# Wu-sm/Adversarial-Attacks-on-GAN-based-Image-Fusion

Measured on AMD Instinct MI355X. Metric: attacked images/sec, PGD-20 L∞ ε=8/255 at 256², 1/2/4/8 MI355X, higher is better.
Workload: dtype f32; 1 GPU; PGD-20 L∞ eps=8/255 alpha=2/255 at 256², 128 images/GPU (BASELINE config #4 per-GPU share), RCCL all-gather of outputs when N>1; encoder=e4e, norm=linf, images_per_gpu=128, global_batch=128, size=256, pgd_steps=20, parallelism=dp1, dist_world_size=1, output_in_eps_ball_and_finite=True, fp32_arithmetic=fp32

## Files before the change

### adversarial-attacks-on-gan-based-image-fusion_amd/csrc/conv_halo_x6.hip

```cpp
#include <type_traits>

#include "conv_common.h"
#include "halo_epilogue.h"

namespace mia {

#ifdef MIA_STAMPS
__device__ unsigned long long g_x6_stamps[4][24];
#endif

template <int BN_, int TPS_ = 1>
struct HaloX6 {
  static constexpr int PH = 16, PW = 16, NW = 8, NT = 64 * NW;
  static constexpr int WN = BN_ == 128 ? 2 : 1, WM = NW / WN, FM = 16 / WM, FN = 4;
  static constexpr int BM = PH * PW, BN = BN_, BK = 32;
  static constexpr int HSIDE = PW + 2, HROWS = (PH + 2) * HSIDE;
  static constexpr int HPIECES = (HROWS + 7) / 8;
  static constexpr int HBUF = HPIECES * 1024;
  static constexpr int LROWB = 64, LBUF = HROWS * LROWB;
  static constexpr int TPS = TPS_, NG = (9 + TPS - 1) / TPS;
  static constexpr int BHM = BN * ROWB, BL = BN * LROWB, BSTAGE1 = BHM + BL;
  static constexpr int BSTAGE = TPS * BSTAGE1;
  static constexpr int BWAVES = 4, HWAVES = 4;
  static constexpr int B_HM_INS = BN / 8 / BWAVES;
// ... 2 lines not shown
  static constexpr int HSTEPS = (4 + TPS - 1) / TPS;
  static constexpr int H_PER_STEP = (H_INS + HSTEPS - 1) / HSTEPS;
  static constexpr int EROWS = 128, ES = BN + 4;
  static constexpr int LDS = 2 * HBUF + LBUF + 2 * BSTAGE;
  static_assert(WM * FM * 16 == BM && WN * FN * 16 == BN, "");
  static_assert(B_HM_INS * 8 * BWAVES == BN && B_L_INS * 16 * BWAVES == BN, "");
  static_assert(LDS <= 160 * 1024, "");
};

template <int BN_, bool PRO, int EPI, bool EARLY, bool PRIO, bool UNR, int TPS = 1, int STG = 0>
__global__ __launch_bounds__(HaloX6<BN_>::NT, 2) void conv_halo_x6_kernel(const ConvK k) {
  static_assert(!UNR || (EARLY && PRIO && EPI != -2), "UNR: the EARLY + PRIO schedule, D[ch][px]");
  static_assert(UNR || TPS == 1, "several taps per K-step: the unrolled loop only");
  static_assert(STG == 0 || (UNR && TPS == 1 && BN_ == 128), "staggered loop: the 128-column tile");
  typedef HaloX6<BN_, TPS> TL;
  constexpr int NG = TL::NG;
  constexpr int FM = TL::FM, FN = TL::FN, WN = TL::WN, NT = TL::NT, BN = TL::BN, BK = TL::BK;
  constexpr int HSIDE = TL::HSIDE, HROWS = TL::HROWS, HPIECES = TL::HPIECES, HBUF = TL::HBUF;
  constexpr int H_INS = TL::H_INS, HPS = TL::H_PER_STEP, HWAVES = TL::HWAVES;
  constexpr int B_HM_INS = TL::B_HM_INS, B_L_INS = TL::B_L_INS, BSTAGE = TL::BSTAGE;

  extern __shared__ __attribute__((aligned(16))) char smem[];
  char* const hbuf = smem;
  char* const lbuf = smem + 2 * HBUF;
  char* const bring = lbuf + TL::LBUF;

  const mia_conv_args& p = k.a;
  const int tid = threadIdx.x, lane = tid & 63;
  const int wid = __builtin_amdgcn_readfirstlane(tid >> 6);
  const int wm = wid / WN, wn = wid % WN;
  const ConvGroup G = k.g[0];
  const int H = p.H, W = p.W, Cin = p.Cin, Cout = p.Cout, Kpad = G.kpad;
  const int bl = xcd_remap(blockIdx.x, k.nblk);
  const int mt = bl / k.nbn, n0 = (bl % k.nbn) * BN;
  const int ptx = W / TL::PW, pty = H / TL::PH;
  const int x0 = (mt % ptx) * TL::PW;
  const int y0 = ((mt / ptx) % pty) * TL::PH;
  const int n = mt / (ptx * pty);

  const float* __restrict__ X = (const float*)p.x;
  const unsigned* __restrict__ Whm = (const unsigned*)G.w_split;
  const __bf16* __restrict__ Wl = (const __bf16*)(Whm + (size_t)Cout * Kpad);
  const char* zero = (const char*)g_zero16;
  const bool bwave = wid < TL::BWAVES;
  const int hw = wid - TL::BWAVES;
  const int my_pieces = bwave ? 0 : (HPIECES - hw + HWAVES - 1) / HWAVES;
#ifdef MIA_STAMPS
  const unsigned long long st_t0 = __builtin_amdgcn_s_memtime();
  const unsigned long long st_r0 = __builtin_amdgcn_s_memrealtime();
  unsigned long long st_pro = 0, st_cv = 0, st_wb = 0;
  unsigned long long st_rd = 0, st_m0 = 0, st_arr = 0, st_rel = 0;
#endif

  constexpr int NSRC = H_INS > B_HM_INS + B_L_INS ? H_INS : B_HM_INS + B_L_INS;
  const char* src[NSRC];
#pragma unroll
  for (int j = 0; j < NSRC; ++j) {
    src[j] = nullptr;
    if (bwave) {
      if (j < B_HM_INS) {
        const int row = (wid * B_HM_INS + j) * 8 + (lane >> 3);
        const int c = EPI >= 0 ? min(n0 + row, Cout - 1) : n0 + row;
        if (c < Cout)
          src[j] = (const char*)(Whm + (size_t)c * Kpad + ((lane & 7) ^ fsw(row)) * 4);
      } else if (j < B_HM_INS + B_L_INS) {
        const int row = (wid * B_L_INS + j - B_HM_INS) * 16 + (lane >> 2);
        const int c = EPI >= 0 ? min(n0 + row, Cout - 1) : n0 + row;
        if (c < Cout)
          src[j] = (const char*)(Wl + (size_t)c * Kpad + ((lane & 3) ^ (lsw(row) >> 1)) * 8);
      }
    } else if (j < H_INS) {
      const int hr = (hw + HWAVES * j) * 8 + (lane >> 3);
      const int hy = hr / HSIDE, hx = hr - (hr / HSIDE) * HSIDE;
      const int y = y0 + hy - 1, x = x0 + hx - 1;
      if (hr < HROWS && y >= 0 && y < H && x >= 0 && x < W)
        src[j] = (const char*)(X + ((size_t)(n * H + y) * W + x) * Cin + ((lane & 7) ^ fsw(hr)) * 4);
    }
  }
  const int ncb = Cin / BK, nk = NG * ncb;

  auto issue_b = [&](int s, int st) {
    const int cb = s / NG, tg = s - (s / NG) * NG;
#pragma unroll
    for (int tt = 0; tt < TPS; ++tt) {
      const int t = tg * TPS + tt;
      if (TPS > 1 && t >= 9) break;
      const int koff = t * Cin + cb * BK;
      char* dst = bring + st * BSTAGE + tt * TL::BSTAGE1;
#pragma unroll
      for (int j = 0; j < B_HM_INS; ++j) {
        const char* a = EPI >= 0 ? src[j] + (size_t)koff * 4
                                 : src[j] ? src[j] + (size_t)koff * 4 : zero;
        __builtin_amdgcn_global_load_lds((gptr_t)a, (lptr_t)(dst + (wid * B_HM_INS + j) * 1024),
                                         16, 0, 0);
      }
#pragma unroll
      for (int j = 0; j < B_L_INS; ++j) {
        const char* a = EPI >= 0                ? src[B_HM_INS + j] + (size_t)koff * 2
                        : src[B_HM_INS + j] ? src[B_HM_INS + j] + (size_t)koff * 2
                                            : zero;
        __builtin_amdgcn_global_load_lds((gptr_t)a,
                                         (lptr_t)(dst + TL::BHM + (wid * B_L_INS + j) * 1024), 16,
                                         0, 0);
      }
    }
  };
  auto issue_h = [&](int cb, int j, int buf) {
    const char* a = src[j] ? src[j] + (size_t)cb * BK * 4 : zero;
    __builtin_amdgcn_global_load_lds((gptr_t)a,
                                     (lptr_t)(hbuf + buf * HBUF + (hw + HWAVES * j) * 1024), 16,
                                     0, 0);
  };
  const bool lrelu_in = p.act_in == MIA_ACT_LRELU_S2;
  auto convert = [&](int cb, int buf) {
    char* hb = hbuf + buf * HBUF;
    for (int c = tid; c < HROWS * 8; c += NT) {
      const int hr = c >> 3, pc = c & 7, lc = pc ^ fsw(hr);
      f32x4 v = *(const f32x4*)(hb + hr * ROWB + pc * 16);
      if constexpr (PRO) {
        const float mul = lrelu_in ? SQRT2 : 1.f;
        f32x4 s4 = {1.f, 1.f, 1.f, 1.f};
        if (p.in_scale) s4 = *(const f32x4*)(p.in_scale + (size_t)n * Cin + cb * BK + lc * 4);
#pragma unroll
        for (int e = 0; e < 4; ++e) {
          float f = v[e];
          if (lrelu_in) f = fmaxf(f, 0.2f * f);
          v[e] = f * (s4[e] * mul);
        }
      }
      u32x4 hm;
      u32x2 lo;
      split_quad(v, hm, lo);
      *(u32x4*)(hb + hr * ROWB + pc * 16) = hm;
      *(u32x2*)(lbuf + hr * TL::LROWB + ((lc ^ lsw(hr)) << 3)) = lo;
    }
  };

  if (bwave) {
    issue_b(0, 0);
  } else {
#pragma unroll
    for (int j = 0; j < H_INS; ++j)
      if (j < my_pieces) issue_h(0, j, 0);
  }
  asm volatile("s_waitcnt vmcnt(0)" ::: "memory");
  __syncthreads();
  convert(0, 0);
  __syncthreads();
#ifdef MIA_STAMPS
  st_pro = __builtin_amdgcn_s_memtime();
#endif

  f32x4 acc[FM][FN];
#pragma unroll
  for (int i = 0; i < FM; ++i)
#pragma unroll
    for (int j = 0; j < FN; ++j) acc[i][j] = f32x4{0.f, 0.f, 0.f, 0.f};

  const int frow = lane & 15, fq = lane >> 4;
  if constexpr (UNR) {
    int oh[FM + 2][3], ol[FM + 2][3];
// ... 306 lines not shown
#ifdef MIA_STAMPS
  if (wid == 0 && lane == 0) {
    const unsigned long long t1 = __builtin_amdgcn_s_memtime();
    const unsigned long long r1 = __builtin_amdgcn_s_memrealtime();
    unsigned long long* g = g_x6_stamps[(BN_ == 128 ? 1 : 0) + (PRO ? 2 : 0)];
    atomicAdd(g + 0, 1ull);
    atomicAdd(g + 1, t1 - st_t0);
    atomicAdd(g + 2, st_pro - st_t0);
    atomicAdd(g + 3, st_cv);
    atomicAdd(g + 4, t1 - st_loop);
    atomicAdd(g + 5, r1 - st_r0);
    atomicAdd(g + 6, (unsigned long long)nk);
    atomicAdd(g + 7, st_wb);
  }
  if (wid == 4 && lane == 0) atomicAdd(&g_x6_stamps[(BN_ == 128 ? 1 : 0) + (PRO ? 2 : 0)][8], st_wb);
  if ((wid == 0 || wid == 4) && lane == 0) {
    unsigned long long* g = g_x6_stamps[(BN_ == 128 ? 1 : 0) + (PRO ? 2 : 0)] + (wid ? 13 : 9);
    atomicAdd(g + 0, st_rd);
    atomicAdd(g + 1, st_m0);
    atomicAdd(g + 2, st_arr);
    atomicAdd(g + 3, st_rel);
  }
#endif
}

template <int BN_, bool PRO, int EPI, bool EARLY, bool PRIO = false, bool UNR = false,
          int TPS = 1, int STG = 0>
static int launch_x6_e(ConvK& k, hipStream_t st) {
  typedef HaloX6<BN_, TPS> TL;
  k.nbn = (k.a.Cout + TL::BN - 1) / TL::BN;
  k.nblk = k.a.N * (k.a.H / TL::PH) * (k.a.W / TL::PW) * k.nbn;
  size_t lds = TL::LDS;
  lds = std::max(lds, (size_t)TL::EROWS * TL::ES * 4);
  lds = std::max(lds, (size_t)TL::NW * TL::BN * 4);
  auto fn = conv_halo_x6_kernel<BN_, PRO, EPI, EARLY, PRIO, UNR, TPS, STG>;
  if (const int rc = ensure_dyn_lds((const void*)fn, 160 * 1024); rc != MIA_OK) return rc;
  k.prered = EPI >= 0 && (EPI & epi::CSUM);
  const int H = k.a.H, W = k.a.W;
  const int nslots = EPI >= 0    ? halo_red_slots(H, W, TL::FM, TL::WM, k.prered)
                     : EPI == -1 ? halo_red_slots(H, W, TL::FM, TL::WM, false)
                                 : (H / TL::PH) * (W / TL::PW);
  RedQ r;
  int rc = conv_red_begin(k, r, nslots, st);
  if (rc != MIA_OK) return rc;
  hipLaunchKernelGGL(fn, dim3(k.nblk), dim3(TL::NT), lds, st, k);
  rc = check_launch("conv_halo_x6");
  return rc != MIA_OK ? rc : red_finish(r, st);
}

constexpr bool x6_stagger_wins(bool pro, int epi) {
#ifdef MIA_X6_STAGGER_ALL
  return MIA_X6_STAGGER_ALL != 0;
#else
  (void)epi;
  return !pro;
#endif
}

template <int BN_, bool PRO, int EPI>
static int launch_x6_(ConvK& k, hipStream_t st) {
  if constexpr (EPI >= 0) {
    const int u = tune(T_X6_UNR);
    if constexpr (BN_ == 64) {
      if (u == 2) return launch_x6_e<BN_, PRO, EPI, true, true, true, 2>(k, st);
    }
    if constexpr (BN_ == 128) {
      const int sg = tune(T_X6_STAGGER);
      if (u != 0 && (sg < 0 ? x6_stagger_wins(PRO, EPI) : sg != 0))
        return launch_x6_e<BN_, PRO, EPI, true, true, true, 1, 1>(k, st);
    }
    if (u != 0) return launch_x6_e<BN_, PRO, EPI, true, true, true>(k, st);
  }
  return launch_x6_e<BN_, PRO, EPI, true, true>(k, st);
}

struct HaloX6S {
  static constexpr int PH = 8, PW = 16, NW = 4, NT = 64 * NW;
  static constexpr int WN = 1, WM = 4, FM = 2, FN = 4;
  static constexpr int BM = PH * PW, BN = 64, BK = 32;
  static constexpr int HSIDE = PW + 2, HROWS = (PH + 2) * HSIDE;
  static constexpr int HPIECES = (HROWS + 7) / 8;
  static constexpr int HBUF = HPIECES * 1024;
  static constexpr int LROWB = 64, LBUF = HROWS * LROWB;
  static constexpr int BHM = BN * ROWB, BL = BN * LROWB, BSTAGE = BHM + BL;
  static constexpr int B_HM_INS = BN / 8 / NW, B_L_INS = BN / 16 / NW;
  static constexpr int H_INS = (HPIECES + NW - 1) / NW;
  static constexpr int EROWS = 128, ES = BN + 4;
  static constexpr int LDS = HBUF + LBUF + 2 * BSTAGE;
  static_assert(WM * FM * 16 == BM && WN * FN * 16 == BN, "");
  static_assert(B_HM_INS * 8 * NW == BN && B_L_INS * 16 * NW == BN, "");
  static_assert(LDS <= 80 * 1024, "two blocks per CU");
};

template <bool PRO, int EPI>
__global__ __launch_bounds__(HaloX6S::NT, 2) void conv_halo_x6s_kernel(const ConvK k) {
  static_assert(EPI >= 0, "the specialised register epilogues only");
  typedef HaloX6S TL;
  constexpr int FM = TL::FM, FN = TL::FN, NT = TL::NT, BN = TL::BN, BK = TL::BK;
  constexpr int HSIDE = TL::HSIDE, HROWS = TL::HROWS, HPIECES = TL::HPIECES;
  constexpr int H_INS = TL::H_INS, B_HM_INS = TL::B_HM_INS, B_L_INS = TL::B_L_INS;
  constexpr int BSTAGE = TL::BSTAGE;

  extern __shared__ __attribute__((aligned(16))) char smem[];
  char* const hbuf = smem;
  char* const lbuf = smem + TL::HBUF;
  char* const bring = lbuf + TL::LBUF;

  const mia_conv_args& p = k.a;
// ... 305 lines not shown
```

### adversarial-attacks-on-gan-based-image-fusion_amd/csrc/conv_upconv.hip

```cpp
#include "conv_common.h"

namespace mia {

template <int BN_>
struct HaloUpT {
  static constexpr int PH = 8, PW = 16, NW = 4, NT = 256;
  static constexpr int WN = BN_ == 64 ? 2 : 1, WM = NW / WN, FM = PH / WM, FN = 2;
  static constexpr int BN = WN * FN * 16;
  static constexpr int HSIDE = PW + 1, HROWS = (PH + 1) * HSIDE;
  static constexpr int HPIECES = (HROWS + 7) / 8;
  static constexpr int HBUF = HPIECES * 8 * ROWB;
  static constexpr int BROWS = 2 * BN, BSTAGE = BROWS * ROWB;
  static constexpr int BWAVES = 2, HWAVES = 2;
  static constexpr int B_INS = BROWS / (8 * BWAVES);
  static constexpr int H_INS = (HPIECES + HWAVES - 1) / HWAVES;
  static constexpr int HPS = (H_INS + 3) / 4;
  static constexpr int NSTEP = 5, STAGES = 2;
  static_assert(B_INS * 8 * BWAVES == BROWS && H_INS * HWAVES == HPIECES, "");
  static_assert(WM * FM == PH && WN * FN * 16 == BN_, "");
};
typedef HaloUpT<64> HaloUp;

__device__ __forceinline__ constexpr int up_jy(int st) { return st == 3 || st == 4 ? 1 : 0; }
__device__ __forceinline__ constexpr int up_jx(int st) { return st == 2 || st == 4 ? 1 : 0; }
__device__ __forceinline__ constexpr int up_phase(int st, int slot) {
  return st == 0 ? slot : st == 1 ? 2 + slot : st == 2 ? 2 * slot : st == 3 ? slot : (slot ? -1 : 0);
}

constexpr int UP_MAX_SRC = 8;
struct UpK {
  const void* x;
  const void* w;
  void* t;
  const float* style;
  const void* mask_a;
  const float* mask_slope;
  int N, R, Cin, Cout, act_in, nbn, nblk, accumulate;
  const void* xs[UP_MAX_SRC];
  int cin_src;
  const void* w_split;
};

__device__ __forceinline__ const char* up_src(const UpK& k, int i) {
  const void* p = k.xs[0];
#pragma unroll
  for (int j = 1; j < UP_MAX_SRC; ++j) p = i == j ? k.xs[j] : p;
  return (const char*)p;
}

template <typename T, bool PRO, bool DG, int BN_ = 64>
__global__ __launch_bounds__(256, 2) void upconv_halo_kernel(const UpK k) {
  typedef HaloUpT<BN_> TL;
// ... 227 lines not shown
        const auto r = __builtin_amdgcn_permlane16_swap(__builtin_bit_cast(unsigned, ta),
                                                        __builtin_bit_cast(unsigned, tb), false,
                                                        false);
        a[h] = r[0];
        b[h] = r[1];
      }
      const int c = n0 + wn * FN * 16 + 16 * (lrow & 1) + 8 * (lrow >> 1);
      const size_t off = ((size_t)(n * TS + ty) * TS + tx) * Cout + c;
      if constexpr (DG) {
        if (k.mask_a || k.accumulate) {
          typedef typename Vec<T>::type VT8;
          VT8 v = __builtin_bit_cast(VT8, make_uint4(a[0], a[1], b[0], b[1]));
          float f[8];
#pragma unroll
          for (int e = 0; e < 8; ++e) f[e] = (float)v[e];
          if (k.mask_a) {
            const VT8 m = *(const VT8*)((const T*)k.mask_a + off);
#pragma unroll
            for (int e = 0; e < 8; ++e) f[e] = (float)m[e] > 0.f ? f[e] : msl[e] * f[e];
          }
          if (k.accumulate) {
            const VT8 o = *(const VT8*)(Y + off);
#pragma unroll
            for (int e = 0; e < 8; ++e) f[e] += (float)o[e];
          }
#pragma unroll
          for (int e = 0; e < 8; ++e) v[e] = (T)f[e];
          *(VT8*)(Y + off) = v;
          continue;
        }
      }
      *(uint4*)(Y + off) = make_uint4(a[0], a[1], b[0], b[1]);
    }
  }
  }
}

template <typename T, bool PRO, bool DG = false, int BN_ = 64>
static int launch_upconv_halo(UpK& k, hipStream_t st) {
  typedef HaloUpT<BN_> TL;
  k.nbn = k.Cout / TL::BN;
  k.nblk = k.N * (k.R / TL::PH) * (k.R / TL::PW) * k.nbn;
  size_t lds = 2 * (size_t)TL::HBUF + (size_t)TL::STAGES * TL::BSTAGE;
  if (PRO) lds += (size_t)k.Cin * sizeof(T);
  if (lds > 160 * 1024) return set_error("upconv_halo: LDS budget exceeded");
  auto fn = upconv_halo_kernel<T, PRO, DG, BN_>;
  if (const int rc = ensure_dyn_lds((const void*)fn, 160 * 1024); rc != MIA_OK) return rc;
  hipLaunchKernelGGL(fn, dim3(k.nblk), dim3(TL::NT), lds, st, k);
  return check_launch("upconv_halo");
}

bool upconv_halo_eligible(int dtype, int R, int Cin, int Cout) {
  if (tune(T_UPCONV_HALO) == 0) return false;
  return R % 16 == 0 && Cin % 64 == 0 && Cout % 32 == 0 &&
         (int64_t)(2 * R + 1) * (2 * R + 1) < (1LL << 31);
}

template <bool DG, bool PRO>
static int launch_upconv_x6(UpK& k, hipStream_t st);
static bool upconv_x6_ok(const UpK& k, int dtype);

int launch_upconv_halo(const void* x, const void* w_up, const void* w_up_split, void* t, int N,
                       int R, int Cin, int Cout, int act_in, const float* style, int dtype,
                       hipStream_t st) {
  UpK k = {};
  k.x = x; k.w = w_up; k.t = t; k.style = style;
  k.N = N; k.R = R; k.Cin = Cin; k.Cout = Cout; k.act_in = act_in;
  k.xs[0] = x; k.cin_src = Cin;
  k.w_split = w_up_split;
  const bool pro = style != nullptr || act_in != MIA_ACT_NONE;
  if (upconv_x6_ok(k, dtype))
    return pro ? launch_upconv_x6<false, true>(k, st) : launch_upconv_x6<false, false>(k, st);
  if (Cout % 64) {
    MIA_DISPATCH_DTYPE(dtype, T, {
      return pro ? launch_upconv_halo<T, true, false, 32>(k, st)
                 : launch_upconv_halo<T, false, false, 32>(k, st);
    });
  }
  MIA_DISPATCH_DTYPE(dtype, T, {
    return pro ? launch_upconv_halo<T, true, false>(k, st)
               : launch_upconv_halo<T, false, false>(k, st);
  });
  return set_error("upconv_halo: unknown dtype");
}

struct DgX6 {
  static constexpr int PH = 16, PW = 16, NW = 8, NT = 64 * NW;
  static constexpr int WM = 4, WN = 2, FM = 4, FN = 2;
  static constexpr int BN = WN * FN * 16, BK = 32;
  static constexpr int HSIDE = PW + 1, HROWS = (PH + 1) * HSIDE;
  static constexpr int HPIECES = (HROWS + 7) / 8;
  static constexpr int HBUF = HPIECES * 1024;
  static constexpr int LROWB = 64, LBUF = HROWS * LROWB;
  static constexpr int BROWS = 2 * BN;
  static constexpr int BHM = BROWS * ROWB, BSTAGE = BHM + BROWS * LROWB;
  static constexpr int BWAVES = 4, HWAVES = 4;
  static constexpr int B_HM_INS = BROWS / 8 / BWAVES;
  static constexpr int B_L_INS = BROWS / 16 / BWAVES;
  static constexpr int H_INS = (HPIECES + HWAVES - 1) / HWAVES;
  static constexpr int HPS = (H_INS + 3) / 4;
  static constexpr int NSTEP = 5;
  static constexpr int LDS = 2 * HBUF + LBUF + 2 * BSTAGE;
  static_assert(WM * FM == PH && WN * FN * 16 == BN, "");
  static_assert(B_HM_INS * 8 * BWAVES == BROWS && B_L_INS * 16 * BWAVES == BROWS, "");
  static_assert(LDS <= 160 * 1024, "");
};

template <bool DG, bool PRO, bool EARLY, bool PRIO>
__global__ __launch_bounds__(DgX6::NT, 1) void upconv_x6_kernel(const UpK k) {
  typedef DgX6 TL;
  constexpr int FM = TL::FM, FN = TL::FN, WN = TL::WN, BN = TL::BN, BK = TL::BK, NT = TL::NT;
  constexpr int HSIDE = TL::HSIDE, HROWS = TL::HROWS, HPIECES = TL::HPIECES, HBUF = TL::HBUF;
  constexpr int H_INS = TL::H_INS, HPS = TL::HPS, HWAVES = TL::HWAVES, BSTAGE = TL::BSTAGE;
  constexpr int B_HM_INS = TL::B_HM_INS, B_L_INS = TL::B_L_INS;

  extern __shared__ __attribute__((aligned(16))) char smem[];
  char* const hbuf = smem;
  char* const lbuf = smem + 2 * HBUF;
  char* const bring = lbuf + TL::LBUF;

  const int tid = threadIdx.x, lane = tid & 63;
  const int wid = __builtin_amdgcn_readfirstlane(tid >> 6);
  const int wm = wid / WN, wn = wid % WN;
  const int R = k.R, Cin = k.Cin, Cout = k.Cout;
  const int bl = xcd_remap(blockIdx.x, k.nblk);
  const int mt = bl / k.nbn, n0 = (bl % k.nbn) * BN;
  const int ptx = R / TL::PW, pty = R / TL::PH;
  const int x0 = (mt % ptx) * TL::PW;
  const int y0 = ((mt / ptx) % pty) * TL::PH;
  const int n = mt / (ptx * pty);
  const int ncb = Cin / BK, nk = TL::NSTEP * ncb;
  const int csrc = k.cin_src, cbs = csrc / BK;
  const char* Whm = (const char*)k.w_split;
  const char* Wl = Whm + (size_t)nk * 2 * Cout * ROWB;
  const size_t hm_step = (size_t)2 * Cout * ROWB, l_step = (size_t)2 * Cout * TL::LROWB;
  const char* zero = (const char*)g_zero16;
  const bool bwave = wid < TL::BWAVES;
  const int hw = wid - TL::BWAVES;

  constexpr int NSRC = H_INS > B_HM_INS + B_L_INS ? H_INS : B_HM_INS + B_L_INS;
  int off[NSRC];
#pragma unroll
  for (int j = 0; j < NSRC; ++j) {
    off[j] = -1;
    if (bwave) {
      if (j < B_HM_INS) {
        const int row = (wid * B_HM_INS + j) * 8 + (lane >> 3);
        const int slot = row / BN, c = n0 + row % BN;
        off[j] = (slot * Cout + c) * ROWB + ((lane & 7) ^ fsw(row)) * 16;
      } else if (j < B_HM_INS + B_L_INS) {
        const int row = (wid * B_L_INS + j - B_HM_INS) * 16 + (lane >> 2);
        const int slot = row / BN, c = n0 + row % BN;
        off[j] = (slot * Cout + c) * TL::LROWB + ((lane & 3) ^ (lsw(row) >> 1)) * 16;
      }
    } else if (j < H_INS) {
      const int hr = (hw + HWAVES * j) * 8 + (lane >> 3);
      const int hy = hr / HSIDE, hx = hr - (hr / HSIDE) * HSIDE;
      const int y = y0 + hy - (DG ? 0 : 1), x = x0 + hx - (DG ? 0 : 1);
      if (hr < HROWS && y >= 0 && y < R && x >= 0 && x < R)
        off[j] = ((n * R + y) * R + x) * csrc + ((lane & 7) ^ fsw(hr)) * 4;
    }
// ... 21 lines not shown
    const int sc = cb / cbs;
    const float* xb = (const float*)up_src(k, sc) + (cb - sc * cbs) * BK;
    const int o = opaque(off[j]);
    const char* a = o >= 0 ? (const char*)(xb + o) : zero;
    __builtin_amdgcn_global_load_lds((gptr_t)a,
                                     (lptr_t)(hbuf + buf * HBUF + (hw + HWAVES * j) * 1024), 16,
                                     0, 0);
  };
  const bool lrelu_in = k.act_in == MIA_ACT_LRELU_S2;
  auto convert = [&](int cb) {
    char* hb = hbuf + (cb & 1) * HBUF;
    for (int c = tid; c < HROWS * 8; c += NT) {
      const int hr = c >> 3, pc = c & 7, lc = pc ^ fsw(hr);
      f32x4 v = *(const f32x4*)(hb + hr * ROWB + pc * 16);
      if constexpr (PRO) {
        const float mul = lrelu_in ? SQRT2 : 1.f;
        f32x4 s4 = {1.f, 1.f, 1.f, 1.f};
        if (k.style) s4 = *(const f32x4*)(k.style + (size_t)n * Cin + cb * BK + lc * 4);
#pragma unroll
        for (int e = 0; e < 4; ++e) {
          float f = v[e];
          if (lrelu_in) f = fmaxf(f, 0.2f * f);
          v[e] = f * (s4[e] * mul);
        }
      }
      u32x4 hm;
      u32x2 lo;
      split_quad(v, hm, lo);
      *(u32x4*)(hb + hr * ROWB + pc * 16) = hm;
      *(u32x2*)(lbuf + hr * TL::LROWB + ((lc ^ lsw(hr)) << 3)) = lo;
    }
  };

  if (bwave) {
    issue_b(0, 0);
  } else {
#pragma unroll
    for (int j = 0; j < H_INS; ++j)
      if (hw + HWAVES * j < HPIECES) issue_h(0, j, 0);
  }
  asm volatile("s_waitcnt vmcnt(0)" ::: "memory");
  __syncthreads();
  convert(0);
  __syncthreads();

  f32x4 acc[4][FM][FN];
#pragma unroll
  for (int q = 0; q < 4; ++q)
#pragma unroll
    for (int i = 0; i < FM; ++i)
#pragma unroll
      for (int j = 0; j < FN; ++j) acc[q][i][j] = f32x4{0.f, 0.f, 0.f, 0.f};

  for (int cb = 0; cb < ncb; ++cb) {
    const char* ha = hbuf + (cb & 1) * HBUF;
#pragma unroll
    for (int st = 0; st < TL::NSTEP; ++st) {
      const int ln = opaque(lane);
      const int frow = ln & 15, fq = ln >> 4;
      const int s = cb * TL::NSTEP + st;
      const char* sb = bring + (s & 1) * BSTAGE;
      if (bwave && s + 1 < nk) issue_b(s + 1, (s & 1) ^ 1);
      const int jy = up_jy(st), jx = up_jx(st);
      if constexpr (EARLY) {
        if (!bwave && st < 4 && cb + 1 < ncb) {
#pragma unroll
          for (int q = 0; q < HPS; ++q) {
            const int j = st * HPS + q;
            if (j < H_INS && hw + HWAVES * j < HPIECES) issue_h(cb + 1, j, (cb + 1) & 1);
          }
        }
      }
#pragma unroll
      for (int h = 0; h < 2; ++h) {
        const int ch = h * 4 + fq;
        u32x4 ahm[FM];
        u32x2 al[FM];
#pragma unroll
        for (int i = 0; i < FM; ++i) {
          const int hr = DG ? (wm * FM + i + jy) * HSIDE + frow + jx
                            : (wm * FM + i + 1 - jy) * HSIDE + frow + 1 - jx;
          ahm[i] = *(const u32x4*)(ha + hr * ROWB + ((ch ^ fsw(hr)) << 4));
          al[i] = *(const u32x2*)(lbuf + hr * TL::LROWB + ((ch ^ lsw(hr)) << 3));
        }
#pragma unroll
        for (int slot = 0; slot < 2; ++slot) {
          const int ph = up_phase(st, slot);
          if (ph < 0) continue;
          u32x4 bhm[FN];
          u32x2 blo[FN];
#pragma unroll
          for (int j = 0; j < FN; ++j) {
            const int row = slot * BN + wn * FN * 16 + 16 * j + frow;
            bhm[j] = *(const u32x4*)(sb + row * ROWB + ((ch ^ fsw(row)) << 4));
            blo[j] = *(const u32x2*)(sb + TL::BHM + row * TL::LROWB + ((ch ^ lsw(row)) << 3));
          }
          if constexpr (PRIO) __builtin_amdgcn_s_setprio(1);
#pragma unroll
          for (int i = 0; i < FM; ++i)
#pragma unroll
            for (int j = 0; j < FN; ++j)
              acc[ph][i][j] = mfma_x6(bhm[j], blo[j], ahm[i], al[i], acc[ph][i][j]);
          if constexpr (PRIO) __builtin_amdgcn_s_setprio(0);
        }
        if (!EARLY && h == 0 && !bwave && st < 4 && cb + 1 < ncb) {
          __builtin_amdgcn_sched_barrier(0);
#pragma unroll
          for (int q = 0; q < HPS; ++q) {
            const int j = st * HPS + q;
            if (j < H_INS && hw + HWAVES * j < HPIECES) issue_h(cb + 1, j, (cb + 1) & 1);
          }
          __builtin_amdgcn_sched_barrier(0);
        }
      }
      if (bwave || st == TL::NSTEP - 1) asm volatile("s_waitcnt vmcnt(0)" ::: "memory");
      __builtin_amdgcn_s_waitcnt(0xc07f);
      __builtin_amdgcn_s_barrier();
      __builtin_amdgcn_sched_barrier(0);
      if (st == TL::NSTEP - 1 && cb + 1 < ncb) {
        convert(cb + 1);
        __syncthreads();
      }
    }
  }

  const int frow = lane & 15, fq = lane >> 4;
  float* __restrict__ Y = (float*)k.t;
  const int TS = DG ? 2 * R : 2 * R + 1;
  float msl[FN][4];
#pragma unroll
  for (int j = 0; j < FN; ++j)
#pragma unroll
    for (int e = 0; e < 4; ++e)
      msl[j][e] = k.mask_slope ? k.mask_slope[n0 + wn * FN * 16 + 16 * j + 4 * fq + e] : 0.f;
#pragma unroll
  for (int ph = 0; ph < 4; ++ph) {
    const int py = ph >> 1, px = ph & 1;
#pragma unroll
    for (int i = 0; i < FM; ++i) {
      const int ty = 2 * (y0 + wm * FM + i) + (DG ? 1 - py : py);
      const int tx = 2 * (x0 + frow) + (DG ? 1 - px : px);
#pragma unroll
      for (int j = 0; j < FN; ++j) {
        const int c = n0 + wn * FN * 16 + 16 * j + 4 * fq;
        const size_t o = ((size_t)(n * TS + ty) * TS + tx) * Cout + c;
        f32x4 v = acc[ph][i][j];
        if (DG && k.mask_a) {
          const f32x4 m = *(const f32x4*)((const float*)k.mask_a + o);
#pragma unroll
          for (int e = 0; e < 4; ++e) v[e] = m[e] > 0.f ? v[e] : msl[j][e] * v[e];
        }
        if (DG && k.accumulate) {
          const f32x4 a = *(const f32x4*)(Y + o);
#pragma unroll
          for (int e = 0; e < 4; ++e) v[e] += a[e];
        }
        *(f32x4*)(Y + o) = v;
      }
    }
  }
}

struct DgX6S {
  static constexpr int PH = 8, PW = 16, NW = 4, NT = 64 * NW;
  static constexpr int WM = 4, WN = 1, FM = 2, FN = 4;
  static constexpr int BN = WN * FN * 16, BK = 32;
  static constexpr int HSIDE = PW + 1, HROWS = (PH + 1) * HSIDE;
  static constexpr int HPIECES = (HROWS + 7) / 8;
  static constexpr int HBUF = HPIECES * 1024;
  static constexpr int LROWB = 64, LBUF = HROWS * LROWB;
  static constexpr int BROWS = 2 * BN;
  static constexpr int BHM = BROWS * ROWB, BSTAGE = BHM + BROWS * LROWB;
  static constexpr int B_HM_INS = BROWS / 8 / NW;
  static constexpr int B_L_INS = BROWS / 16 / NW;
  static constexpr int H_INS = (HPIECES + NW - 1) / NW;
  static constexpr int NSTEP = 5;
// ... 175 lines not shown
      convert(cb + 1);
      __syncthreads();
    }
  }

  const int frow = lane & 15, fq = lane >> 4;
  float* __restrict__ Y = (float*)k.t;
  const int TS = DG ? 2 * R : 2 * R + 1;
  float msl[FN][4];
#pragma unroll
  for (int j = 0; j < FN; ++j)
#pragma unroll
    for (int e = 0; e < 4; ++e)
      msl[j][e] = k.mask_slope ? k.mask_slope[n0 + wn * FN * 16 + 16 * j + 4 * fq + e] : 0.f;
#pragma unroll
  for (int ph = 0; ph < 4; ++ph) {
    const int py = ph >> 1, px = ph & 1;
#pragma unroll
    for (int i = 0; i < FM; ++i) {
      const int ty = 2 * (y0 + wm * FM + i) + (DG ? 1 - py : py);
      const int tx = 2 * (x0 + frow) + (DG ? 1 - px : px);
#pragma unroll
      for (int j = 0; j < FN; ++j) {
        const int c = n0 + wn * FN * 16 + 16 * j + 4 * fq;
        const size_t o = ((size_t)(n * TS + ty) * TS + tx) * Cout + c;
        f32x4 v = acc[ph][i][j];
        if (DG && k.mask_a) {
          const f32x4 m = *(const f32x4*)((const float*)k.mask_a + o);
#pragma unroll
          for (int e = 0; e < 4; ++e) v[e] = m[e] > 0.f ? v[e] : msl[j][e] * v[e];
        }
        if (DG && k.accumulate) {
          const f32x4 a = *(const f32x4*)(Y + o);
#pragma unroll
          for (int e = 0; e < 4; ++e) v[e] += a[e];
        }
        *(f32x4*)(Y + o) = v;
      }
    }
  }
}

template <bool DG, bool PRO>
static int launch_upconv_x6s(UpK& k, hipStream_t st) {
  typedef DgX6S TL;
  k.nbn = k.Cout / TL::BN;
  k.nblk = k.N * (k.R / TL::PH) * (k.R / TL::PW) * k.nbn;
  auto fn = upconv_x6s_kernel<DG, PRO>;
  if (const int rc = ensure_dyn_lds((const void*)fn, 80 * 1024); rc != MIA_OK) return rc;
  hipLaunchKernelGGL(fn, dim3(k.nblk), dim3(TL::NT), TL::LDS, st, k);
  return check_launch("upconv_x6s");
}

template <bool DG, bool PRO, bool EARLY, bool PRIO>
static int launch_upconv_x6_e(UpK& k, hipStream_t st) {
  typedef DgX6 TL;
  k.nbn = k.Cout / TL::BN;
  k.nblk = k.N * (k.R / TL::PH) * (k.R / TL::PW) * k.nbn;
  auto fn = upconv_x6_kernel<DG, PRO, EARLY, PRIO>;
  if (const int rc = ensure_dyn_lds((const void*)fn, 160 * 1024); rc != MIA_OK) return rc;
  hipLaunchKernelGGL(fn, dim3(k.nblk), dim3(TL::NT), TL::LDS, st, k);
  return check_launch("upconv_x6");
}

template <bool DG, bool PRO>
static int launch_upconv_x6(UpK& k, hipStream_t st) {
  if (DG && tune(T_UPCONV_X6S) != 0 && k.Cin <= 512) return launch_upconv_x6s<DG, PRO>(k, st);
  return launch_upconv_x6_e<DG, PRO, true, false>(k, st);
}

static bool upconv_x6_ok(const UpK& k, int dtype) {
#ifdef MIA_F32_NATIVE
  (void)k;
  (void)dtype;
  return false;
#else
  if (tune(T_UPCONV_X6) == 0) return false;
  return dtype == MIA_F32 && k.w_split && k.R % DgX6::PH == 0 && k.Cout % DgX6::BN == 0 &&
         k.Cin % DgX6::BK == 0;
#endif
}

static bool s2dg_x6_ok(const UpK& k, int dtype) {
#ifdef MIA_F32_NATIVE
  (void)k;
  (void)dtype;
  return false;
#else
  if (tune(T_S2DG_X6) == 0) return false;
  return dtype == MIA_F32 && k.w_split && k.R % DgX6::PH == 0 && k.Cout % DgX6::BN == 0 &&
         k.cin_src % DgX6::BK == 0;
#endif
}

bool s2_dgrad_halo_eligible(int dtype, int R, int Cg, int Cx) {
  if (tune(T_S2DG_HALO) == 0) return false;
  (void)dtype;
  return R % 16 == 0 && Cg % 64 == 0 && Cx % HaloUp::BN == 0 &&
         (int64_t)4 * R * R < (1LL << 31);
}

}

using namespace mia;

extern "C" int mia_conv_s2_dgrad_halo_multi(const void* const* g, int ng, const void* w_halo,
                                            const void* w_split, void* gx, int N, int R, int Cg,
                                            int Cx, const void* mask_a, const float* mask_slope,
                                            int accumulate, int dtype, void* stream) {
  MIA_CHECK_ARG(g && ng >= 1 && ng <= UP_MAX_SRC && w_halo && gx && N > 0, "bad args");
  for (int i = 0; i < ng; ++i) MIA_CHECK_ARG(g[i], "null source tensor");
  MIA_CHECK_ARG(s2_dgrad_halo_eligible(dtype, R, Cg, Cx),
                "needs R % 16 == 0, Cg % 64 == 0, Cx % 64 == 0 "
                "(use mia_conv2d phase groups otherwise)");
  MIA_CHECK_ARG((int64_t)N * R * R * Cg < (1LL << 31), "input too large for 32-bit offsets");
  UpK k = {};
  k.x = g[0]; k.w = w_halo; k.t = gx; k.mask_a = mask_a; k.mask_slope = mask_slope;
  k.N = N; k.R = R; k.Cin = ng * Cg; k.Cout = Cx; k.accumulate = accumulate;
  for (int i = 0; i < ng; ++i) k.xs[i] = g[i];
  k.cin_src = Cg;
  k.w_split = w_split;
  if (s2dg_x6_ok(k, dtype)) return launch_upconv_x6<true, false>(k, (hipStream_t)stream);
  MIA_DISPATCH_DTYPE(dtype, T, return launch_upconv_halo<T, false, true>(k, (hipStream_t)stream));
  return set_error("s2_dgrad_halo: unknown dtype");
}


extern "C" int mia_conv_s2_dgrad_halo(const void* g, const void* w_halo, void* gx, int N, int R,
                                      int Cg, int Cx, const void* mask_a, const float* mask_slope,
                                      int accumulate, int dtype, void* stream) {
  const void* gs[1] = {g};
  return mia_conv_s2_dgrad_halo_multi(gs, 1, w_halo, nullptr, gx, N, R, Cg, Cx, mask_a,
                                      mask_slope, accumulate, dtype, stream);
}
```

### adversarial-attacks-on-gan-based-image-fusion_amd/csrc/mia_common.h

```cpp
#pragma once
#include <hip/hip_runtime.h>
#include <stdint.h>
#include <string>

#include "../../include/miattack.h"

namespace mia {

typedef __attribute__((ext_vector_type(4))) float f32x4;
typedef __attribute__((ext_vector_type(8))) _Float16 f16x8;
typedef __attribute__((ext_vector_type(8))) __bf16 bf16x8;

template <typename T> struct Vec;
template <> struct Vec<float> { typedef f32x4 type; static constexpr int N = 4; };
template <> struct Vec<_Float16> { typedef f16x8 type; static constexpr int N = 8; };
template <> struct Vec<__bf16> { typedef bf16x8 type; static constexpr int N = 8; };

__device__ __forceinline__ float to_f(float v) { return v; }
__device__ __forceinline__ float to_f(_Float16 v) { return (float)v; }
__device__ __forceinline__ float to_f(__bf16 v) { return (float)v; }
template <typename T> __device__ __forceinline__ T from_f(float v);
template <> __device__ __forceinline__ float from_f<float>(float v) { return v; }
template <> __device__ __forceinline__ _Float16 from_f<_Float16>(float v) { return (_Float16)v; }
template <> __device__ __forceinline__ __bf16 from_f<__bf16>(float v) { return (__bf16)v; }
// ... 3 lines not shown
__device__ __forceinline__ float lrelu_s2(float v) { return (v > 0.f ? v : 0.2f * v) * SQRT2; }
__device__ __forceinline__ float lrelu_s2_grad(float pre) { return pre > 0.f ? SQRT2 : 0.2f * SQRT2; }
__device__ __forceinline__ float lrelu_s2_inv_grad(float pre) {
  return pre > 0.f ? 0.70710678118654752f : 3.5355339059327376f;
}

#define MIA_DPP(v, ctrl) \
  __builtin_bit_cast(float, __builtin_amdgcn_mov_dpp(__builtin_bit_cast(int, (v)), (ctrl), 0xf, 0xf, false))
__device__ __forceinline__ void lds_handoff() {
  asm volatile("s_waitcnt lgkmcnt(0)\n\ts_barrier" ::: "memory");
}

__device__ __forceinline__ float row16_sum(float v) {
  v += MIA_DPP(v, 0xB1);
  v += MIA_DPP(v, 0x4E);
  v += MIA_DPP(v, 0x141);
  v += MIA_DPP(v, 0x140);
  return v;
}

__device__ __forceinline__ float wave_sum(float v) {
#pragma unroll
  for (int o = 32; o > 0; o >>= 1) v += __shfl_xor(v, o, 64);
  return v;
}

int set_error(const std::string& msg);
int check_launch(const char* what);

int device_cu_count();
int ensure_dyn_lds(const void* fn, int bytes);
int max_blocks_per_cu(const void* fn, int threads, size_t dyn_lds);

enum TuneKey {
  T_CONV_HALO,
  T_CONV_X6,
  T_HALO_EPI,
  T_X6_UNR,
  T_CONV_THIN,
  T_CONV_THIN32,
  T_CONV_WRES,
  T_CONV_REGEPI,
  T_CONV_SMALLTILE,
  T_S2DG_X6,
  T_S2DG_HALO,
  T_UPCONV_X6,
  T_UPCONV_HALO,
  T_CONV_WRES32,
  T_HALO_C64,
  T_X6_64S,
  T_UPCONV_X6S,
  T_CONV_WRES128,
  T_X6_STAGGER,
  T_NKEYS
};
int tune(TuneKey key);

struct RedQ {
  float* dst[3];
  float* part;
  int nslots, count;
};
float* red_scratch(hipStream_t st, size_t bytes);
int red_begin(RedQ& r, float* d0, float* d1, float* d2, int nslots, int count, hipStream_t st,
              bool zero = false);
int red_finish(const RedQ& r, hipStream_t st);

__device__ __forceinline__ void red_store(float* part, int nslots, int count, int q, int slot,
                                          int i, float v) {
  part[((size_t)q * nslots + slot) * count + i] = v;
}

}

#define MIA_DISPATCH_DTYPE(dtype, T, ...)                                   \
  switch (dtype) {                                                          \
    case MIA_F32: { typedef float T; __VA_ARGS__; break; }                  \
    case MIA_F16: { typedef _Float16 T; __VA_ARGS__; break; }               \
    case MIA_BF16: { typedef __bf16 T; __VA_ARGS__; break; }                \
    default: return mia::set_error("unsupported dtype");                    \
  }

#define MIA_CHECK_ARG(cond, msg) \
  do { if (!(cond)) return mia::set_error(std::string(__func__) + ": " + (msg)); } while (0)
```

### adversarial-attacks-on-gan-based-image-fusion_amd/csrc/reduce.hip

```cpp
#include <algorithm>
#include <cstdlib>
#include <cstring>
#include <mutex>
#include <unordered_map>
#include <vector>

#include "mia_common.h"

namespace mia {

namespace {
struct Scratch {
  float* p = nullptr;
  size_t bytes = 0;
};
std::mutex g_mu;
std::unordered_map<hipStream_t, Scratch> g_scratch;
}

namespace {
struct TuneDef {
  const char* name;
  int value;
};
TuneDef g_tune[T_NKEYS] = {
    {"MIA_CONV_HALO", 1}, {"MIA_CONV_X6", 1},       {"MIA_HALO_EPI", 1},    {"MIA_X6_UNR", 2},
    {"MIA_CONV_THIN", 1}, {"MIA_CONV_THIN32", 1},   {"MIA_CONV_WRES", 1},
    {"MIA_CONV_REGEPI", 1},   {"MIA_CONV_SMALLTILE", 512},
    {"MIA_S2DG_X6", 1},   {"MIA_S2DG_HALO", 1},     {"MIA_UPCONV_X6", 1},   {"MIA_UPCONV_HALO", 1},
    {"MIA_CONV_WRES32", 1},
    {"MIA_HALO_C64", 1},  {"MIA_X6_64S", 1},
    {"MIA_UPCONV_X6S", 1}, {"MIA_CONV_WRES128", 1}, {"MIA_X6_STAGGER", -1}};
std::once_flag g_tune_once;
void tune_init() {
  for (auto& d : g_tune) {
    if (&d == &g_tune[T_X6_STAGGER]) continue;
    const char* e = getenv(d.name);
    if (e && *e) d.value = atoi(e);
  }
}
}

int tune(TuneKey key) {
  std::call_once(g_tune_once, tune_init);
  return g_tune[key].value;
}

namespace {
std::mutex g_dev_mu;
std::unordered_map<int, int> g_ncu;
std::unordered_map<const void*, std::vector<int>> g_lds_set;
int current_device() {
  int dev = 0;
  (void)hipGetDevice(&dev);
  return dev;
}
}

int device_cu_count() {
  const int dev = current_device();
  std::lock_guard<std::mutex> lock(g_dev_mu);
  auto it = g_ncu.find(dev);
  if (it != g_ncu.end()) return it->second;
  int ncu = 0;
  if (hipDeviceGetAttribute(&ncu, hipDeviceAttributeMultiprocessorCount, dev) != hipSuccess ||
      ncu <= 0)
    ncu = 256;
  g_ncu[dev] = ncu;
  return ncu;
}

int ensure_dyn_lds(const void* fn, int bytes) {
  const int dev = current_device();
  std::lock_guard<std::mutex> lock(g_dev_mu);
  std::vector<int>& done = g_lds_set[fn];
  if (std::find(done.begin(), done.end(), dev) != done.end()) return MIA_OK;
  if (hipFuncSetAttribute(fn, hipFuncAttributeMaxDynamicSharedMemorySize, bytes) != hipSuccess)
    return set_error("hipFuncSetAttribute(MaxDynamicSharedMemorySize) failed");
  done.push_back(dev);
  return MIA_OK;
}

int max_blocks_per_cu(const void* fn, int threads, size_t dyn_lds) {
  static std::unordered_map<const void*, std::unordered_map<int, int>> cache;
  const int dev = current_device();
  std::lock_guard<std::mutex> lock(g_dev_mu);
  auto& per_dev = cache[fn];
  auto it = per_dev.find(dev);
  if (it != per_dev.end()) return it->second;
// ... 173 lines not shown
```

### adversarial-attacks-on-gan-based-image-fusion_amd/layouts.py

```python
import weakref

import torch

BLUR_F = (0.25, 0.75, 0.75, 0.25)


def kpad_for(cin, dtype):
    bk = 32 if dtype == torch.float32 else 64
    return (9 * cin + bk - 1) // bk * bk


def fwd_matrix(w, dtype, cin_pad=None):
    cout, cin = w.shape[:2]
    cp = cin_pad or cin
    wp = torch.zeros(cout, cp, 3, 3, dtype=torch.float64)
    wp[:, :cin] = w.double()
    m = wp.permute(0, 2, 3, 1).reshape(cout, 9 * cp)
    out = torch.zeros(cout, kpad_for(cp, dtype), dtype=torch.float64)
    out[:, :9 * cp] = m
    return out.to(dtype)


def dgrad_matrix(w, dtype, cin_pad=None):
    cout, cin = w.shape[:2]
    cp = cin_pad or cin
    wt = torch.zeros(cp, cout, 3, 3, dtype=torch.float64)
    wt[:cin] = w.double().transpose(0, 1).flip(2, 3)
    return fwd_matrix(wt, dtype)


def upconv_subpixel_matrices(w, dtype):
    cout, cin = w.shape[:2]
    w = w.double()
    out = []
    for ph in range(4):
        py, px = ph >> 1, ph & 1
        kh, kw = 2 - py, 2 - px
        m = torch.zeros(cout, kh, kw, cin, dtype=torch.float64)
        for ty in range(kh):
            for tx in range(kw):
                m[:, ty, tx, :] = w[:, :, py + 2 * (kh - 1 - ty), px + 2 * (kw - 1 - tx)]
        bk = 32 if dtype == torch.float32 else 64
        kp = (kh * kw * cin + bk - 1) // bk * bk
        full = torch.zeros(cout, kp, dtype=torch.float64)
        full[:, :kh * kw * cin] = m.reshape(cout, -1)
        out.append(full.to(dtype))
    return out


UPCONV_HALO_STEPS = (((0, 0), (0, 1)), ((0, 0), (2, 3)), ((0, 1), (0, 2)), ((1, 0), (0, 1)),
                     ((1, 1), (0, None)))


def halo_bk(dtype):
    return 32 if dtype == torch.float32 else 64


def upconv_halo_matrix(w, dtype):
    cout, cin = w.shape[:2]
    if cin % 64:
        raise ValueError("Cin must be a multiple of 64")
    bk = halo_bk(dtype)
    w = w.double()
    out = torch.zeros(cin // bk, 5, 2, cout, bk, dtype=torch.float64)
    for st, ((jy, jx), phases) in enumerate(UPCONV_HALO_STEPS):
        for slot, ph in enumerate(phases):
            if ph is None:
                continue
            py, px = ph >> 1, ph & 1
            wk = w[:, :, py + 2 * jy, px + 2 * jx]
            out[:, st, slot] = wk.reshape(cout, cin // bk, bk).permute(1, 0, 2)
    return out.to(dtype)


def upconv_dgrad_matrix(w, dtype):
    return fwd_matrix(w.double().transpose(0, 1), dtype)


def upconv_phases(w):
    cout, cin = w.shape[:2]
    w = w.double()
    v = torch.zeros(2, 2, cout, cin, 3, 3, dtype=torch.float64)
    for py in range(2):
        for px in range(2):
            for ty in range(3):
                for tx in range(3):
                    acc = torch.zeros(cout, cin, dtype=torch.float64)
                    for jy in range(4):
                        ky = 1 - 2 * ty + py + jy
                        if not 0 <= ky <= 2:
                            continue
                        for jx in range(4):
                            kx = 1 - 2 * tx + px + jx
                            if not 0 <= kx <= 2:
                                continue
                            acc += BLUR_F[jy] * BLUR_F[jx] * w[:, :, ky, kx]
                    v[py, px, :, :, ty, tx] = acc
    return v.reshape(4 * cout, cin, 3, 3)


S2_KMAP = ((1,), (2, 0))


def s2_dgrad_phases(w, dtype):
    cout, cin = w.shape[:2]
    w = w.double()
    bk = 32 if dtype == torch.float32 else 64
    out = []
    for ph in range(4):
        py, px = ph >> 1, ph & 1
        ky, kx = S2_KMAP[py], S2_KMAP[px]
        m = torch.zeros(cin, len(ky), len(kx), cout, dtype=torch.float64)
        for ty, a in enumerate(ky):
            for tx, b in enumerate(kx):
                m[:, ty, tx, :] = w[:, :, a, b].t()
# ... 69 lines not shown
```

Measured before the change: 17.73 attacked images/s.

## Stagger weight and halo waves in upconv x6 kernel and extend stagger to prologue convs

Adds a staggered schedule to the upconv bf16x6 kernel. Weight-loading waves run ahead while halo waves lag by one step and interleave their next-chunk halo loads with MFMAs. The halo conv kernel now enables stagger by default for prologue variants too, and recomputes halo source addresses at issue time to cut register pressure. It also relaxes the fp32 Cin eligibility for upconv and s2-dgrad halo paths to multiples of 32, which routes more layers to the halo kernels. The risk is extra address arithmetic and schedule imbalance between the two wave groups.

```diff
diff --git a/adversarial-attacks-on-gan-based-image-fusion_amd/csrc/conv_halo_x6.hip b/adversarial-attacks-on-gan-based-image-fusion_amd/csrc/conv_halo_x6.hip
--- a/adversarial-attacks-on-gan-based-image-fusion_amd/csrc/conv_halo_x6.hip
+++ b/adversarial-attacks-on-gan-based-image-fusion_amd/csrc/conv_halo_x6.hip
@@ -78,7 +78,8 @@
   unsigned long long st_rd = 0, st_m0 = 0, st_arr = 0, st_rel = 0;
 #endif
 
-  constexpr int NSRC = H_INS > B_HM_INS + B_L_INS ? H_INS : B_HM_INS + B_L_INS;
+  constexpr bool HRE = STG != 0 && PRO;
+  constexpr int NSRC = !HRE && H_INS > B_HM_INS + B_L_INS ? H_INS : B_HM_INS + B_L_INS;
   const char* src[NSRC];
 #pragma unroll
   for (int j = 0; j < NSRC; ++j) {
@@ -95,7 +96,7 @@
         if (c < Cout)
           src[j] = (const char*)(Wl + (size_t)c * Kpad + ((lane & 3) ^ (lsw(row) >> 1)) * 8);
       }
-    } else if (j < H_INS) {
+    } else if (!HRE && j < H_INS) {
       const int hr = (hw + HWAVES * j) * 8 + (lane >> 3);
       const int hy = hr / HSIDE, hx = hr - (hr / HSIDE) * HSIDE;
       const int y = y0 + hy - 1, x = x0 + hx - 1;
@@ -132,7 +133,20 @@
     }
   };
   auto issue_h = [&](int cb, int j, int buf) {
-    const char* a = src[j] ? src[j] + (size_t)cb * BK * 4 : zero;
+    const char* a;
+    if constexpr (HRE) {
+      int ln = lane;
+      asm volatile("" : "+v"(ln));
+      const int hr = (hw + HWAVES * j) * 8 + (ln >> 3);
+      const int hy = hr / HSIDE, hx = hr - (hr / HSIDE) * HSIDE;
+      const int y = y0 + hy - 1, x = x0 + hx - 1;
+      a = zero;
+      if (hr < HROWS && y >= 0 && y < H && x >= 0 && x < W)
+        a = (const char*)(X + ((size_t)(n * H + y) * W + x) * Cin + ((ln & 7) ^ fsw(hr)) * 4) +
+            (size_t)cb * BK * 4;
+    } else {
+      a = src[j] ? src[j] + (size_t)cb * BK * 4 : zero;
+    }
     __builtin_amdgcn_global_load_lds((gptr_t)a,
                                      (lptr_t)(hbuf + buf * HBUF + (hw + HWAVES * j) * 1024), 16,
                                      0, 0);
@@ -545,8 +559,9 @@
 #ifdef MIA_X6_STAGGER_ALL
   return MIA_X6_STAGGER_ALL != 0;
 #else
+  (void)pro;
   (void)epi;
-  return !pro;
+  return true;
 #endif
 }
 
diff --git a/adversarial-attacks-on-gan-based-image-fusion_amd/csrc/conv_upconv.hip b/adversarial-attacks-on-gan-based-image-fusion_amd/csrc/conv_upconv.hip
--- a/adversarial-attacks-on-gan-based-image-fusion_amd/csrc/conv_upconv.hip
+++ b/adversarial-attacks-on-gan-based-image-fusion_amd/csrc/conv_upconv.hip
@@ -1,3 +1,5 @@
+#include <type_traits>
+
 #include "conv_common.h"
 
 namespace mia {
@@ -331,7 +333,7 @@
 
 bool upconv_halo_eligible(int dtype, int R, int Cin, int Cout) {
   if (tune(T_UPCONV_HALO) == 0) return false;
-  return R % 16 == 0 && Cin % 64 == 0 && Cout % 32 == 0 &&
+  return R % 16 == 0 && Cin % (dtype == MIA_F32 ? 32 : 64) == 0 && Cout % 32 == 0 &&
          (int64_t)(2 * R + 1) * (2 * R + 1) < (1LL << 31);
 }
 
@@ -385,7 +387,7 @@
   static_assert(LDS <= 160 * 1024, "");
 };
 
-template <bool DG, bool PRO, bool EARLY, bool PRIO>
+template <bool DG, bool PRO, bool EARLY, bool PRIO, int STG = 0>
 __global__ __launch_bounds__(DgX6::NT, 1) void upconv_x6_kernel(const UpK k) {
   typedef DgX6 TL;
   constexpr int FM = TL::FM, FN = TL::FN, WN = TL::WN, BN = TL::BN, BK = TL::BK, NT = TL::NT;
@@ -513,6 +515,94 @@
 #pragma unroll
       for (int j = 0; j < FN; ++j) acc[q][i][j] = f32x4{0.f, 0.f, 0.f, 0.f};
 
+  if constexpr (STG != 0) {
+    auto loop = [&](auto lagc) {
+      constexpr bool lag = decltype(lagc)::value;
+      u32x4 ahm[FM], bhm[2][FN];
+      u32x2 al[FM], blo[2][FN];
+      auto mfmas = [&](int stp) __attribute__((always_inline)) {
+        if constexpr (PRIO) __builtin_amdgcn_s_setprio(1);
+#pragma unroll
+        for (int slot = 0; slot < 2; ++slot) {
+          const int ph = up_phase(stp, slot);
+          if (ph < 0) continue;
+#pragma unroll
+          for (int i = 0; i < FM; ++i)
+#pragma unroll
+            for (int j = 0; j < FN; ++j)
+              acc[ph][i][j] = mfma_x6(bhm[slot][j], blo[slot][j], ahm[i], al[i], acc[ph][i][j]);
+        }
+        if constexpr (PRIO) __builtin_amdgcn_s_setprio(0);
+      };
+      for (int cb = 0; cb < ncb; ++cb) {
+        const char* ha = hbuf + (cb & 1) * HBUF;
+#pragma unroll
+        for (int st = 0; st < TL::NSTEP; ++st) {
+          const int ln = opaque(lane);
+          const int frow = ln & 15, fq = ln >> 4;
+          const int s = cb * TL::NSTEP + st;
+          const char* sb = bring + (s & 1) * BSTAGE;
+          if (!lag && s + 1 < nk) issue_b(s + 1, (s & 1) ^ 1);
+          const int jy = up_jy(st), jx = up_jx(st);
+#pragma unroll
+          for (int h = 0; h < 2; ++h) {
+            auto reads = [&]() __attribute__((always_inline)) {
+              const int ch = h * 4 + fq;
+#pragma unroll
+              for (int i = 0; i < FM; ++i) {
+                const int hr = DG ? (wm * FM + i + jy) * HSIDE + frow + jx
+                                  : (wm * FM + i + 1 - jy) * HSIDE + frow + 1 - jx;
+                ahm[i] = *(const u32x4*)(ha + hr * ROWB + ((ch ^ fsw(hr)) << 4));
+                al[i] = *(const u32x2*)(lbuf + hr * TL::LROWB + ((ch ^ lsw(hr)) << 3));
+              }
+#pragma unroll
+              for (int slot = 0; slot < 2; ++slot) {
+                if (up_phase(st, slot) < 0) continue;
+#pragma unroll
+                for (int j = 0; j < FN; ++j) {
+                  const int row = slot * BN + wn * FN * 16 + 16 * j + frow;
+                  bhm[slot][j] = *(const u32x4*)(sb + row * ROWB + ((ch ^ fsw(row)) << 4));
+                  blo[slot][j] =
+                      *(const u32x2*)(sb + TL::BHM + row * TL::LROWB + ((ch ^ lsw(row)) << 3));
+                }
+              }
+            };
+            if constexpr (!lag) {
+              reads();
+              mfmas(st);
+            } else {
+              if (h == 1) mfmas(st);
+              else if (st > 0) mfmas(st - 1);
+              if (h == 0 && st < 4 && cb + 1 < ncb) {
+#pragma unroll
+                for (int q = 0; q < HPS; ++q) {
+                  const int j = st * HPS + q;
+                  if (j < H_INS && hw + HWAVES * j < HPIECES) issue_h(cb + 1, j, (cb + 1) & 1);
+                }
+              }
+              reads();
+            }
+          }
+          if (!lag || st == TL::NSTEP - 1) asm volatile("s_waitcnt vmcnt(0)" ::: "memory");
+          lds_handoff();
+          __builtin_amdgcn_sched_barrier(0);
+          if (st == TL::NSTEP - 1) {
+            if constexpr (lag) {
+              mfmas(st);
+              __builtin_amdgcn_sched_barrier(0);
+            }
+            if (cb + 1 < ncb) {
+              convert(cb + 1);
+              __syncthreads();
+            }
+          }
+        }
+      }
+    };
+    static_assert(TL::BWAVES == 4, "the weight waves lead, the halo waves lag");
+    if (bwave) loop(std::false_type{});
+    else loop(std::true_type{});
+  } else {
   for (int cb = 0; cb < ncb; ++cb) {
     const char* ha = hbuf + (cb & 1) * HBUF;
 #pragma unroll
@@ -583,6 +673,7 @@
         __syncthreads();
       }
     }
+  }
   }
 
   const int frow = lane & 15, fq = lane >> 4;
@@ -864,20 +955,34 @@
   return check_launch("upconv_x6s");
 }
 
-template <bool DG, bool PRO, bool EARLY, bool PRIO>
+template <bool DG, bool PRO, bool EARLY, bool PRIO, int STG = 0>
 static int launch_upconv_x6_e(UpK& k, hipStream_t st) {
   typedef DgX6 TL;
   k.nbn = k.Cout / TL::BN;
   k.nblk = k.N * (k.R / TL::PH) * (k.R / TL::PW) * k.nbn;
-  auto fn = upconv_x6_kernel<DG, PRO, EARLY, PRIO>;
+  auto fn = upconv_x6_kernel<DG, PRO, EARLY, PRIO, STG>;
   if (const int rc = ensure_dyn_lds((const void*)fn, 160 * 1024); rc != MIA_OK) return rc;
   hipLaunchKernelGGL(fn, dim3(k.nblk), dim3(TL::NT), TL::LDS, st, k);
   return check_launch("upconv_x6");
 }
 
+#ifndef MIA_UPX6_STG_PRIO
+#define MIA_UPX6_STG_PRIO 1
+#endif
+constexpr bool upx6_stagger_wins(bool dg, bool pro) {
+#ifdef MIA_UPX6_STAGGER_ALL
+  return MIA_UPX6_STAGGER_ALL != 0;
+#else
+  return dg || pro;
+#endif
+}
+
 template <bool DG, bool PRO>
 static int launch_upconv_x6(UpK& k, hipStream_t st) {
   if (DG && tune(T_UPCONV_X6S) != 0 && k.Cin <= 512) return launch_upconv_x6s<DG, PRO>(k, st);
+  const int sg = tune(T_UPX6_STAGGER);
+  if (sg < 0 ? upx6_stagger_wins(DG, PRO) : sg != 0)
+    return launch_upconv_x6_e<DG, PRO, true, MIA_UPX6_STG_PRIO != 0, 1>(k, st);
   return launch_upconv_x6_e<DG, PRO, true, false>(k, st);
 }
 
@@ -907,8 +1012,7 @@
 
 bool s2_dgrad_halo_eligible(int dtype, int R, int Cg, int Cx) {
   if (tune(T_S2DG_HALO) == 0) return false;
-  (void)dtype;
-  return R % 16 == 0 && Cg % 64 == 0 && Cx % HaloUp::BN == 0 &&
+  return R % 16 == 0 && Cg % (dtype == MIA_F32 ? 32 : 64) == 0 && Cx % HaloUp::BN == 0 &&
          (int64_t)4 * R * R < (1LL << 31);
 }
 
@@ -923,7 +1027,7 @@
   MIA_CHECK_ARG(g && ng >= 1 && ng <= UP_MAX_SRC && w_halo && gx && N > 0, "bad args");
   for (int i = 0; i < ng; ++i) MIA_CHECK_ARG(g[i], "null source tensor");
   MIA_CHECK_ARG(s2_dgrad_halo_eligible(dtype, R, Cg, Cx),
-                "needs R % 16 == 0, Cg % 64 == 0, Cx % 64 == 0 "
+                "needs R % 16 == 0, Cg % 64 == 0 (fp32: % 32), Cx % 64 == 0 "
                 "(use mia_conv2d phase groups otherwise)");
   MIA_CHECK_ARG((int64_t)N * R * R * Cg < (1LL << 31), "input too large for 32-bit offsets");
   UpK k = {};
diff --git a/adversarial-attacks-on-gan-based-image-fusion_amd/csrc/mia_common.h b/adversarial-attacks-on-gan-based-image-fusion_amd/csrc/mia_common.h
--- a/adversarial-attacks-on-gan-based-image-fusion_amd/csrc/mia_common.h
+++ b/adversarial-attacks-on-gan-based-image-fusion_amd/csrc/mia_common.h
@@ -79,6 +79,7 @@
   T_UPCONV_X6S,
   T_CONV_WRES128,
   T_X6_STAGGER,
+  T_UPX6_STAGGER,
   T_NKEYS
 };
 int tune(TuneKey key);
diff --git a/adversarial-attacks-on-gan-based-image-fusion_amd/csrc/reduce.hip b/adversarial-attacks-on-gan-based-image-fusion_amd/csrc/reduce.hip
--- a/adversarial-attacks-on-gan-based-image-fusion_amd/csrc/reduce.hip
+++ b/adversarial-attacks-on-gan-based-image-fusion_amd/csrc/reduce.hip
@@ -30,11 +30,13 @@
     {"MIA_S2DG_X6", 1},   {"MIA_S2DG_HALO", 1},     {"MIA_UPCONV_X6", 1},   {"MIA_UPCONV_HALO", 1},
     {"MIA_CONV_WRES32", 1},
     {"MIA_HALO_C64", 1},  {"MIA_X6_64S", 1},
-    {"MIA_UPCONV_X6S", 1}, {"MIA_CONV_WRES128", 1}, {"MIA_X6_STAGGER", -1}};
+    {"MIA_UPCONV_X6S", 1}, {"MIA_CONV_WRES128", 1}, {"MIA_X6_STAGGER", -1},
+    {"MIA_UPX6_STAGGER", -1}};
 std::once_flag g_tune_once;
 void tune_init() {
   for (auto& d : g_tune) {
-    if (&d == &g_tune[T_X6_STAGGER]) continue;
+    if (&d == &g_tune[T_X6_STAGGER] || &d == &g_tune[T_UPX6_STAGGER])
+      continue;
     const char* e = getenv(d.name);
     if (e && *e) d.value = atoi(e);
   }
diff --git a/adversarial-attacks-on-gan-based-image-fusion_amd/layouts.py b/adversarial-attacks-on-gan-based-image-fusion_amd/layouts.py
--- a/adversarial-attacks-on-gan-based-image-fusion_amd/layouts.py
+++ b/adversarial-attacks-on-gan-based-image-fusion_amd/layouts.py
@@ -58,9 +58,9 @@
 
 def upconv_halo_matrix(w, dtype):
     cout, cin = w.shape[:2]
-    if cin % 64:
-        raise ValueError("Cin must be a multiple of 64")
     bk = halo_bk(dtype)
+    if cin % bk:
+        raise ValueError(f"Cin must be a multiple of {bk}")
     w = w.double()
     out = torch.zeros(cin // bk, 5, 2, cout, bk, dtype=torch.float64)
     for st, ((jy, jx), phases) in enumerate(UPCONV_HALO_STEPS):
```

Result: no change. 17.87 attacked images/s, median of 6 (+0.8%).
